# aipixel/GPS-Gaussian

Measured on NVIDIA H100. Metric: novel_views_per_sec_1024sq_500kgauss, higher is better.
Workload: dtype f32

## Files before the change

gps-gaussian_b200/csrc/gpsg_capi.cu:

```cuda
#include <cstdarg>
#include <cstdio>
#include <cstring>
#include <cstdlib>
#include "gpsg_internal.cuh"

namespace gpsg {

static thread_local char g_err[1024] = "";

void set_error(const char* fmt, ...) {
    va_list ap;
    va_start(ap, fmt);
    vsnprintf(g_err, sizeof(g_err), fmt, ap);
    va_end(ap);
}

Camera make_camera(const GpsgRasterSettings& s) {
    Camera c;
    memcpy(c.view, s.viewmatrix, sizeof(c.view));
    memcpy(c.proj, s.projmatrix, sizeof(c.proj));
    c.tanfovx = s.tanfovx;
    c.tanfovy = s.tanfovy;
    c.W = s.image_width;
    c.H = s.image_height;
    c.focal_x = (float)c.W / (2.0f * s.tanfovx);
    c.focal_y = (float)c.H / (2.0f * s.tanfovy);
    c.scale_modifier = s.scale_modifier;
    c.grid_x = (c.W + GPSG_TILE_X - 1) / GPSG_TILE_X;
    c.grid_y = (c.H + GPSG_TILE_Y - 1) / GPSG_TILE_Y;
    for (int k = 0; k < 3; ++k) { c.bg[k] = s.bg[k]; c.campos[k] = s.campos[k]; }
    return c;
}

template <typename T>
static inline T* take(char*& p, size_t count) {
    T* r = reinterpret_cast<T*>(p);
    p += align_up(count * sizeof(T));
    return r;
}

static GeomState carve_geom(char* p, int P, size_t scan_bytes, char** end) {
    GeomState g;
    const size_t n = (size_t)(P > 0 ? P : 1);
    g.depths = take<float>(p, n);
    g.means2D = take<float2>(p, n);
    g.conic_opacity = take<float4>(p, n);
    g.rgb = take<float>(p, 3 * n);
    g.clamped = take<uint8_t>(p, 3 * n);
    g.tiles_touched = take<uint32_t>(p, n);
    g.point_offsets = take<uint32_t>(p, n);
    g.scan_temp = p;
    g.scan_temp_bytes = scan_bytes;
    p += align_up(scan_bytes);
    if (end) *end = p;
    return g;
}
size_t GeomState::required(int P, size_t scan_bytes) {
    char* end = nullptr;
    carve_geom(nullptr, P, scan_bytes, &end);
    return (size_t)(end - (char*)nullptr) + 256;
}
GeomState GeomState::carve(void* base, int P, size_t scan_bytes) {
    return carve_geom((char*)align_up((size_t)base), P, scan_bytes, nullptr);
}

static BinningState carve_binning(char* p, size_t N, size_t sort_bytes, char** end) {
    BinningState b;
    const size_t n = N > 0 ? N : 1;
    b.slabA = take<float4>(p, n);
    b.slabB = take<float4>(p, n);
    b.slabC = take<float4>(p, n);
    b.keys = take<uint64_t>(p, n);
    b.vals = take<uint32_t>(p, n);
    b.keys_unsorted = take<uint64_t>(p, n);
    b.bucket = reinterpret_cast<uint2*>(b.keys_unsorted);
    b.vals_unsorted = take<uint32_t>(p, n);
    b.blk_list = take<uint32_t>(p, 8 * n);
    b.sort_temp = p;
    b.sort_temp_bytes = sort_bytes;
    p += align_up(sort_bytes);
    if (end) *end = p;
    return b;
}
size_t BinningState::required(size_t N, size_t sort_bytes) {
    char* end = nullptr;
    carve_binning(nullptr, N, sort_bytes, &end);
    return (size_t)(end - (char*)nullptr) + 256;
}
BinningState BinningState::carve(void* base, size_t N, size_t sort_bytes) {
    return carve_binning((char*)align_up((size_t)base), N, sort_bytes, nullptr);
}

static ImageState carve_image(char* p, int W, int H, char** end) {
    ImageState im;
    const size_t hw = (size_t)W * H;
    const size_t tiles = (size_t)((W + GPSG_TILE_X - 1) / GPSG_TILE_X) * ((H + GPSG_TILE_Y - 1) / GPSG_TILE_Y);
    im.final_T = take<float>(p, hw > 0 ? hw : 1);
    im.n_contrib = take<uint32_t>(p, hw > 0 ? hw : 1);
    im.ranges = take<uint2>(p, tiles > 0 ? tiles : 1);
    im.tile_count = take<uint32_t>(p, tiles > 0 ? tiles : 1);
    im.totals = take<uint32_t>(p, 64);
    im.tile_cursor = take<uint32_t>(p, tiles > 0 ? tiles : 1);
    im.big_tiles = take<uint32_t>(p, tiles > 0 ? tiles : 1);
    im.tile_order = take<uint32_t>(p, tiles > 0 ? tiles : 1);
    im.blk_count = take<uint32_t>(p, 8 * (tiles > 0 ? tiles : 1));
    if (end) *end = p;
    return im;
}
size_t ImageState::required(int W, int H) {
    char* end = nullptr;
    carve_image(nullptr, W, H, &end);
    return (size_t)(end - (char*)nullptr) + 256;
}
ImageState ImageState::carve(void* base, int W, int H) { return carve_image((char*)align_up((size_t)base), W, H, nullptr); }


static GaussianSrc aos_src(const float* means3D, const float* scales, const float* rots, const float* opacities,
                           const float* colors, const float* cov3D_precomp) {
    GaussianSrc src;
    memset(&src, 0, sizeof(src));
    src.means3D = means3D; src.scales = scales; src.rots = rots; src.opacities = opacities; src.colors = colors;
    src.cov3D_precomp = cov3D_precomp;
    return src;
}

static int bit_length(uint32_t n) {
    int b = 0;
    while (n) { ++b; n >>= 1; }
    return b;
}

static bool force_radix_binning() {
    static const bool v = [] { const char* e = getenv("GPSG_BINNING"); return e && e[0] == 'r'; }();
    return v;
}

static uint32_t* pinned_slot() {
    static thread_local uint32_t* slot = nullptr;
    if (!slot) {
        if (cudaHostAlloc((void**)&slot, 64, cudaHostAllocDefault) != cudaSuccess) slot = nullptr;
    }
    return slot;
}

}


#include <mutex>
#include <vector>
namespace gpsg {
struct ProfSlot { cudaEvent_t a, b; Stage stage; bool used; };
struct Profiler {
    int on = 0;
    std::vector<ProfSlot> slots;
    size_t next = 0;
    int launches[ST_COUNT] = {0};
};
static Profiler g_prof;
static std::mutex g_prof_mu;
static const char* kStageNames[ST_COUNT] = {"preprocess", "scan", "duplicate", "sort", "gather_ranges", "tile_scan",
                                            "bucket_scatter", "tile_sort_gather", "render_forward",
                                            "render_backward", "preprocess_backward", "corr_forward", "corr_backward", "corr_build",
                                            "render_backward_det", "render_backward_det_reduce"};
StageTimer::StageTimer(Stage s, cudaStream_t st, int launches) : stage(s), stream(st), slot(nullptr) {
    if (!g_prof.on) return;
    std::lock_guard<std::mutex> lk(g_prof_mu);
    if (g_prof.on == 2) { g_prof.launches[s] += launches; return; }
    if (g_prof.next == g_prof.slots.size()) {
        ProfSlot ps; ps.used = false;
        if (cudaEventCreate(&ps.a) != cudaSuccess || cudaEventCreate(&ps.b) != cudaSuccess) return;
        g_prof.slots.push_back(ps);
    }
    ProfSlot* p = &g_prof.slots[g_prof.next++];
    p->stage = s; p->used = true;
    g_prof.launches[s] += launches;
    cudaEventRecord(p->a, stream);
    slot = (void*)(uintptr_t)(g_prof.next);
}
StageTimer::~StageTimer() {
    if (!slot) return;
    std::lock_guard<std::mutex> lk(g_prof_mu);
    cudaEventRecord(g_prof.slots[(size_t)(uintptr_t)slot - 1].b, stream);
}
}

using namespace gpsg;

extern "C" {

GPSG_API const char* gpsg_last_error(void) { return g_err; }
int gpsg_version(void) { return 90; }

static int forward_exact_begin(const GpsgRasterSettings* s, int device, cudaStream_t stream, int P, const GaussianSrc& src,
                               int32_t* radii, gpsg_alloc_fn geom_alloc, void* geom_user, gpsg_alloc_fn image_alloc,
                               void* image_user, uint32_t* totals_host, void** geom_out, void** image_out, int flags) {
    GPSG_CUDA(cudaSetDevice(device));
    const Camera cam = make_camera(*s);
    const size_t scan_bytes = scan_temp_bytes(P);
    void* geom_base = geom_alloc(geom_user, GeomState::required(P, scan_bytes));
    if (!geom_base) { set_error("geometry allocator returned NULL"); return GPSG_E_ALLOC; }
    GeomState g = GeomState::carve(geom_base, P, scan_bytes);
    void* img_base = image_alloc(image_user, ImageState::required(cam.W, cam.H));
    if (!img_base) { set_error("image allocator returned NULL"); return GPSG_E_ALLOC; }
    ImageState im = ImageState::carve(img_base, cam.W, cam.H);
    if (geom_out) *geom_out = geom_base;
    if (image_out) *image_out = img_base;
    int rc = GPSG_OK;
    GPSG_CUDA(cudaMemsetAsync(im.tile_count, 0, (size_t)((char*)(im.totals + 64) - (char*)im.tile_count), stream));
    if (P > 0) {
        { StageTimer t(ST_PREPROCESS, stream, 1); rc = launch_preprocess(cam, P, src, radii, g, im, 0u, flags, stream); }
        if (rc) return rc;
        GPSG_CUDA(cudaMemcpyAsync(totals_host, im.totals, 6 * sizeof(uint32_t), cudaMemcpyDeviceToHost, stream));
    } else {
        { StageTimer t(ST_TILE_SCAN, stream, 1); rc = launch_tile_scan(cam, im, 0u, stream); }
        if (rc) return rc;
        for (int k = 0; k < 6; ++k) totals_host[k] = 0u;
    }
    return GPSG_OK;
}

static int forward_exact_finish(const GpsgRasterSettings* s, int device, cudaStream_t stream, int P, int sh_M, GaussianSrc src,
                                const float* shs, float* out_color, float* out_depth, float* out_alpha, int32_t* radii,
                                void* geom_base, void* img_base,
                                gpsg_alloc_fn binning_alloc, void* binning_user, const uint32_t* totals_host,
                                int32_t* num_rendered) {
    GPSG_CUDA(cudaSetDevice(device));
    const Camera cam = make_camera(*s);
    GeomState g = GeomState::carve(geom_base, P, scan_temp_bytes(P));
    ImageState im = ImageState::carve(img_base, cam.W, cam.H);
    const int tiles = cam.grid_x * cam.grid_y;
    const uint32_t N = totals_host[0], max_count = totals_host[1];
    GPSG_REQUIRE(totals_host[5] == 0u, "more than 2^31 (tile, Gaussian) pairs: the splats cover (almost) the whole image each -- "
                                       "degenerate scene (32-bit pair offsets, as in the upstream rasterizer)");
    int rc = GPSG_OK;
    if (num_rendered) *num_rendered = (int32_t)N;
    if (shs && P > 0) {
        rc = launch_sh_forward(P, s->sh_degree, sh_M, s->campos, src.means3D, shs, radii, g.rgb, g.clamped, stream);
        if (rc) return rc;
        src.colors = g.rgb;
    }

    const bool radix_path = max_count > kMaxTileSort || force_radix_binning();
    const int end_bit = 32 + bit_length((uint32_t)tiles);
    const size_t sort_bytes = radix_path ? sort_temp_bytes(N, end_bit) : 0;
    void* bin_base = binning_alloc(binning_user, BinningState::required(N, sort_bytes));
    if (!bin_base) { set_error("binning allocator returned NULL"); return GPSG_E_ALLOC; }
    BinningState b = BinningState::carve(bin_base, N, sort_bytes);

    if (N > 0 && !radix_path) {
        { StageTimer t(ST_SCATTER, stream, 1); rc = launch_bucket_scatter(cam, P, radii, g, b, im, stream); }
        if (rc) return rc;
        { StageTimer t(ST_TILE_SORT, stream, max_count > 2048 ? 2 : 1); rc = launch_tile_sort_gather(cam, P, max_count, src, g, b, im, stream); }
        if (rc) return rc;
    } else if (N > 0) {
        { StageTimer t(ST_SCAN, stream, 2); rc = run_scan(g, P, stream); }
        if (rc) return rc;
        { StageTimer t(ST_DUPLICATE, stream, 1); rc = launch_duplicate(cam, P, radii, g, b, stream); }
        if (rc) return rc;
        { StageTimer t(ST_SORT, stream, 2 + (end_bit + 7) / 8); rc = run_sort(b, N, end_bit, stream); }
        if (rc) return rc;
        { StageTimer t(ST_GATHER, stream, 2); rc = launch_gather_ranges(cam, N, src, g, b, im, stream); }
        if (rc) return rc;
    }
    { StageTimer t(ST_RENDER_FWD, stream, 1); rc = launch_render_forward(cam, b, im, out_color, g.depths, out_depth, out_alpha, stream); }
    if (rc) return rc;
    if (s->debug) GPSG_CUDA(cudaStreamSynchronize(stream));
    return GPSG_OK;
}

static int check_fwd_flags(int flags) {
    GPSG_REQUIRE((flags & ~GPSG_FWD_ANTIALIAS) == 0, "unknown forward flag bits (GPSG_FWD_ANTIALIAS is the only flag)");
    return GPSG_OK;
}

static int check_aux_outputs(const float* out_depth, const float* out_alpha) {
    GPSG_REQUIRE((out_depth == nullptr) == (out_alpha == nullptr), "out_depth and out_alpha must both be NULL or both be set");
    return GPSG_OK;
}

int gpsg_rasterize_forward(const GpsgRasterSettings* s, int device, void* stream_, int P, int sh_M,
                           const float* means3D, const float* colors_precomp, const float* shs,
                           const float* opacities, const float* scales, const float* rotations,
                           const float* cov3D_precomp, float* out_color, float* out_depth, float* out_alpha,
                           int32_t* radii, gpsg_alloc_fn geom_alloc, void* geom_user, gpsg_alloc_fn binning_alloc,
                           void* binning_user, gpsg_alloc_fn image_alloc, void* image_user, int32_t* num_rendered,
                           int flags) {
    if (int rc_f = check_fwd_flags(flags)) return rc_f;
    GPSG_REQUIRE(s != nullptr, "settings is NULL");
    GPSG_REQUIRE(P >= 0, "P < 0");
    GPSG_REQUIRE(s->image_width > 0 && s->image_height > 0, "image size must be positive");
    GPSG_REQUIRE(out_color != nullptr, "out_color is NULL");
    if (int rc_aux = check_aux_outputs(out_depth, out_alpha)) return rc_aux;
    GPSG_REQUIRE(geom_alloc && binning_alloc && image_alloc, "allocator callback is NULL");
    if (P > 0) {
        GPSG_REQUIRE(means3D && opacities && radii, "means3D / opacities / radii is NULL");
        GPSG_REQUIRE((colors_precomp != nullptr) != (shs != nullptr),
                     "Please provide excatly one of either SHs or precomputed colors!");
        GPSG_REQUIRE(((scales != nullptr && rotations != nullptr) != (cov3D_precomp != nullptr)),
                     "Please provide exactly one of either scale/rotation pair or precomputed 3D covariance!");
        if (shs) {
            GPSG_REQUIRE(s->sh_degree >= 0 && s->sh_degree <= 3, "sh_degree must be 0..3");
// ... 655 lines not shown
```

gps-gaussian_b200/csrc/gpsg_internal.cuh:

```cuda
#pragma once
#include <cuda_runtime.h>
#include <stdint.h>
#include <stddef.h>
#include "../../include/gpsg.h"

#define GPSG_TILE_X 16
#define GPSG_TILE_Y 16
#define GPSG_TILE_PIX 256

namespace gpsg {

void set_error(const char* fmt, ...);

#define GPSG_CUDA(expr)                                                                         \
    do {                                                                                        \
        cudaError_t _e = (expr);                                                                \
        if (_e != cudaSuccess) {                                                                \
            gpsg::set_error("%s:%d: %s -> %s", __FILE__, __LINE__, #expr, cudaGetErrorString(_e)); \
            return GPSG_E_CUDA;                                                                 \
        }                                                                                       \
    } while (0)
#define GPSG_LAUNCH_CHECK() GPSG_CUDA(cudaGetLastError())
#define GPSG_REQUIRE(cond, msg)                                  \
    do {                                                         \
        if (!(cond)) {                                           \
            gpsg::set_error("%s:%d: %s", __FILE__, __LINE__, msg); \
            return GPSG_E_INVALID;                               \
        }                                                        \
    } while (0)

struct Camera {
    float view[16];
    float proj[16];
    float tanfovx, tanfovy, focal_x, focal_y;
    float scale_modifier;
    int W, H, grid_x, grid_y;
    float bg[3];
    float campos[3];
};
Camera make_camera(const GpsgRasterSettings& s);


struct GaussianSrc {
    const float* means3D; const float* scales; const float* rots; const float* opacities; const float* colors;
    const float* cov3D_precomp;
    int S2;
    const uint8_t* valid[2]; const float* xyz[2]; const float* img[2]; const float* rot[2]; const float* scale[2];
    const float* opac[2];
};
struct GaussianGrads {
    float* dmeans3D; float* dscales; float* drots; float* dopacity; float* dcov3D;
    float* dxyz[2]; float* dimg[2]; float* drot[2]; float* dscale[2]; float* dopac[2];
};
#ifdef __CUDACC__
__device__ __forceinline__ bool src_geom(const GaussianSrc& s, int i, float& x, float& y, float& z, float sc[3], float4& q,
                                         float& op) {
    if (s.S2 == 0) {
        const float* m = s.means3D + 3 * (size_t)i;
        x = m[0]; y = m[1]; z = m[2];
        if (!s.cov3D_precomp) {
            const float* sp = s.scales + 3 * (size_t)i;
            sc[0] = sp[0]; sc[1] = sp[1]; sc[2] = sp[2];
            const float* rp = s.rots + 4 * (size_t)i;
            q = ((reinterpret_cast<uintptr_t>(s.rots) & 15) == 0) ? __ldg(reinterpret_cast<const float4*>(rp))
                                                                   : make_float4(rp[0], rp[1], rp[2], rp[3]);
        }
        op = s.opacities[i];
        return true;
    }
    const int v = i >= s.S2 ? 1 : 0, px = i - v * s.S2;
    if (!s.valid[v][px]) return false;
    const float* xyz = s.xyz[v] + 3 * (size_t)px;
    x = xyz[0]; y = xyz[1]; z = xyz[2];
    const size_t S2 = (size_t)s.S2;
    sc[0] = s.scale[v][px]; sc[1] = s.scale[v][S2 + px]; sc[2] = s.scale[v][2 * S2 + px];
    q = make_float4(s.rot[v][px], s.rot[v][S2 + px], s.rot[v][2 * S2 + px], s.rot[v][3 * S2 + px]);
    op = s.opac[v][px];
    return true;
}
__device__ __forceinline__ void tile_rect(int grid_x, int grid_y, float2 p, int radius, int& rx0, int& ry0, int& rx1,
                                          int& ry1) {
    const float rad = (float)radius;
    rx0 = min(grid_x, max(0, (int)((p.x - rad) / (float)GPSG_TILE_X)));
    ry0 = min(grid_y, max(0, (int)((p.y - rad) / (float)GPSG_TILE_Y)));
    rx1 = min(grid_x, max(0, (int)((p.x + rad + (float)(GPSG_TILE_X - 1)) / (float)GPSG_TILE_X)));
    ry1 = min(grid_y, max(0, (int)((p.y + rad + (float)(GPSG_TILE_Y - 1)) / (float)GPSG_TILE_Y)));
}
__device__ __forceinline__ int fwd_block_col(int k) { return (k >> 1) & 1; }
__device__ __forceinline__ int fwd_block_row(int k) { return ((k >> 2) << 1) + (k & 1); }
__device__ __forceinline__ void fwd_block_origin(int tile_x, int tile_y, int k, int& bx0, int& by0) {
    bx0 = tile_x * GPSG_TILE_X + (fwd_block_col(k) << 3);
    by0 = tile_y * GPSG_TILE_Y + (fwd_block_row(k) << 2);
}
__device__ __forceinline__ void src_color(const GaussianSrc& s, uint32_t id, float& r, float& g, float& b) {
    if (s.S2 == 0) { r = s.colors[3 * id]; g = s.colors[3 * id + 1]; b = s.colors[3 * id + 2]; return; }
    const int v = (int)id >= s.S2 ? 1 : 0;
    const size_t px = id - (uint32_t)(v * s.S2), S2 = (size_t)s.S2;
    r = s.img[v][px] * 0.5f + 0.5f; g = s.img[v][S2 + px] * 0.5f + 0.5f; b = s.img[v][2 * S2 + px] * 0.5f + 0.5f;
}
#endif

static inline size_t align_up(size_t v, size_t a = 256) { return (v + a - 1) / a * a; }

struct GeomState {
    float* depths;
    float2* means2D;
    float4* conic_opacity;
    float* rgb;
    uint8_t* clamped;
    uint32_t* tiles_touched;
    uint32_t* point_offsets;
    void* scan_temp;
    size_t scan_temp_bytes;
    static size_t required(int P, size_t scan_temp_bytes);
    static GeomState carve(void* base, int P, size_t scan_temp_bytes);
};
struct BinningState {
    uint2* bucket;
    uint64_t* keys_unsorted;
    uint32_t* vals_unsorted;
    uint64_t* keys;
    uint32_t* vals;
    float4* slabA;
    float4* slabB;
    float4* slabC;
    uint32_t* blk_list;
    void* sort_temp;
    size_t sort_temp_bytes;
    static size_t required(size_t N, size_t sort_temp_bytes);
    static BinningState carve(void* base, size_t N, size_t sort_temp_bytes);
};
struct ImageState {
    float* final_T;
    uint32_t* n_contrib;
    uint2* ranges;
    uint32_t* tile_count;
    uint32_t* tile_cursor;
    uint32_t* totals;
    uint32_t* big_tiles;
    uint32_t* tile_order;
    uint32_t* blk_count;
    static size_t required(int W, int H);
    static ImageState carve(void* base, int W, int H);
};
constexpr int kFwdFlagsWord = 6;
size_t scan_temp_bytes(int P);
size_t sort_temp_bytes(size_t N, int end_bit);

int launch_preprocess(const Camera& cam, int P, const GaussianSrc& src, int32_t* radii, GeomState g, ImageState im,
                      uint32_t capacity, int fwd_flags, cudaStream_t stream);
int launch_mark_visible(int P, const float* means3D, const float* view16_host, uint8_t* present, cudaStream_t stream);
int run_scan(GeomState g, int P, cudaStream_t stream);
int launch_duplicate(const Camera& cam, int P, const int32_t* radii, GeomState g, BinningState b, cudaStream_t stream);
int run_sort(BinningState b, size_t N, int end_bit, cudaStream_t stream);
int launch_gather_ranges(const Camera& cam, size_t N, const GaussianSrc& src, GeomState g, BinningState b, ImageState im,
                         cudaStream_t stream);
constexpr uint32_t kMaxTileSort = 4096;
int launch_tile_scan(const Camera& cam, ImageState im, uint32_t capacity , cudaStream_t stream);
int launch_bucket_scatter(const Camera& cam, int P, const int32_t* radii, GeomState g, BinningState b, ImageState im,
                          cudaStream_t stream);
int launch_tile_sort_gather(const Camera& cam, int P, uint32_t max_count, const GaussianSrc& src, GeomState g,
                            BinningState b, ImageState im, cudaStream_t stream);
int launch_render_forward(const Camera& cam, BinningState b, ImageState im, float* out_color, const float* depths,
                          float* out_depth, float* out_alpha, cudaStream_t stream);
struct AuxGrads {
    const float* depths; const float* dL_ddepth; const float* dL_dalpha;
    bool on() const { return dL_ddepth != nullptr; }
};
int launch_render_backward(const Camera& cam, BinningState b, ImageState im, const float* dL_dpix, float4* grad_acc,
                           const AuxGrads& aux, cudaStream_t stream);
int launch_render_backward_det(const Camera& cam, BinningState b, ImageState im, const float* dL_dpix, float* det_part,
                               uint32_t* det_mask, const AuxGrads& aux, cudaStream_t stream);
int launch_det_reduce(const Camera& cam, int P, const int32_t* radii, GeomState g, BinningState b, ImageState im,
                      const uint8_t* det_mask, const float* det_part, float4* grad_acc, bool aux, cudaStream_t stream);
int launch_preprocess_backward(const Camera& cam, int P, const GaussianSrc& src, const int32_t* radii,
                               const float4* conic_opacity, const uint32_t* fwd_flags ,
                               const float4* grad_acc, float* dL_dmeans2D ,
                               float* dL_dcolors , const GaussianGrads& out, bool aux,
                               cudaStream_t stream);
int launch_sh_forward(int P, int deg, int M, const float* campos3, const float* means3D, const float* shs,
                      const int32_t* radii, float* rgb, uint8_t* clamped, cudaStream_t stream);
int launch_sh_backward(int P, int deg, int M, const float* campos3, const float* means3D, const float* shs,
                       const int32_t* radii, const uint8_t* clamped, const float* dL_dcolors, float* dL_dsh,
                       float* dL_dmeans3D, cudaStream_t stream);
int launch_unproject_fwd(int B, int S, const float* flow, const float* mask, int64_t mask_bs, const float* intr,
                         const float* extr, int extr_rows, const float* ref_intr, const float* Tf_x, float* depth,
                         float* xyz, uint8_t* valid, cudaStream_t stream);
int launch_unproject_bwd(int B, int S, const float* depth, const float* mask, int64_t mask_bs, const float* intr,
                         const float* extr, int extr_rows, const float* ref_intr, const float* Tf_x,
                         const float* dL_dxyz, const float* dL_ddepth, float* dL_dflow, cudaStream_t stream);
struct RectifyView {
    double iR[9];
    double fx, fy, cx, cy;
    const uint8_t* img; const uint8_t* mask; const float* depth;
    uint8_t* img_out; uint8_t* mask_out; float* depth_out; float* img_tensor; float* mask_tensor;
};
struct RectifyArgs {
    RectifyView v[2];
    int Hin, Win, C, Cm, H, W;
};
struct RectifyFlowArgs {
    const float* depth[2]; const uint8_t* mask[2]; double* flow[2]; uint8_t* valid[2];
    double offset[2], tf[2];
    int H, W, Cm;
};
int launch_rectify_remap(const GpsgRectifyCamera* cams, int Hin, int Win, int C, int Cm, int H, int W,
                         const GpsgRectifyPlanes* planes, cudaStream_t stream);
int launch_rectify_flow(int H, int W, int Cm, double Tf_x, double cx0, double cx1, const float* const* depth,
                        const uint8_t* const* mask, double* const* flow, uint8_t* const* valid, cudaStream_t stream);
size_t point_splat_workspace_bytes(int B, int res);
int launch_point_splat(int B, int N, int res, int64_t rows, const float* pts, const float* mask, float* depth, float* color,
                       void* workspace, cudaStream_t stream);
size_t mesh_render_workspace_bytes(int num_faces, int64_t max_pixels);
int launch_mesh_render(const GpsgMesh& mesh, const GpsgMeshScene& scene, void* workspace, cudaStream_t stream);
int launch_convex_upsample_fwd(int dtype, int f, int N, int D, int H, int W, const float* flow, const void* mask, float* out,
                               cudaStream_t stream);
size_t convex_upsample_workspace_bytes(int N, int D, int H, int W);
int launch_convex_upsample_bwd(int dtype, int f, int N, int D, int H, int W, const float* flow, const void* mask,
                               const float* grad_out, void* grad_mask, float* grad_flow, void* workspace,
                               cudaStream_t stream);
size_t sequence_loss_workspace_bytes();
size_t gs_head_workspace_bytes(int B, int H, int W);
int launch_gs_head_fwd(int device, int B, int H, int W, const float* src, const float* img, const float* depth,
                       const GpsgGsHeadWeights& wt, float* rot, float* scale, float* opacity, void* workspace,
                       cudaStream_t stream);
size_t gs_head_backward_workspace_bytes(int B, int H, int W);
int launch_gs_head_bwd(int device, int B, int H, int W, const float* src, const float* img, const float* depth,
                       const float* mid, const float* g_rot, const float* g_scale, const float* g_opacity,
                       const GpsgGsHeadWeights& wt, float* d_src, float* d_depth, const GpsgGsHeadGrads& grads,
                       void* workspace, cudaStream_t stream);
int launch_sequence_loss_fwd(const GpsgSeqLossArgs& a, float* stats, void* workspace, cudaStream_t stream);
int launch_sequence_loss_bwd(const GpsgSeqLossArgs& a, const float* grad_loss, const float* stats, cudaStream_t stream);
int corr_build_mode();
void set_corr_build_mode(int m);
int launch_corr_fwd(int dtype, int B, int H, int W1, int W2, const void* vol, int64_t sb, int64_t sh, int64_t sw1,
                    const float* coords, int64_t csb, int r, void* out, cudaStream_t stream);
int launch_corr_bwd(int dtype, int B, int H, int W1, int W2, const float* coords, int64_t csb, const void* gout, int r,
                    void* gvol, cudaStream_t stream);
int launch_corr_build(int dtype, int B, int D, int H, int W1, int W2, const void* f1, const void* f2, void* v0, void* v1,
                      void* v2, void* v3, int levels, cudaStream_t stream);
bool corr_build_tc_supported(int dtype, int D, int W1, int W2, const void* f1, const void* f2, void* const* v, int levels);
int launch_corr_build_tc(int B, int D, int H, int W1, int W2, const void* f1, const void* f2, void* v0, void* v1, void* v2,
                         void* v3, int levels, cudaStream_t stream);
bool corr_build_bwd_tc_supported(int dtype, int D, int W1, int W2, const void* f1, const void* f2, const void* g,
                                 const void* d1, const void* d2);
int launch_corr_build_bwd_tc(int B, int D, int H, int W1, int W2, const void* f1, const void* f2, const void* g, void* df1,
                             void* df2, cudaStream_t stream);
int launch_corr_build_bwd(int dtype, int B, int D, int H, int W1, int W2, const void* f1, const void* f2, const void* g,
                          void* df1, void* df2, cudaStream_t stream);
int launch_corr_lookup_fwd(int dtype, int B, int H, int W1, const void* const* vols, const int* widths, int levels,
                           const float* coords, int64_t csb, int r, void* out, cudaStream_t stream);
int launch_corr_lookup_bwd(int dtype, int B, int H, int W1, void* const* gvols, const int* widths, int levels,
                           const float* coords, int64_t csb, int r, const void* gout, cudaStream_t stream);

size_t l1_ssim_workspace_bytes(int planes, int H, int W);
int launch_l1_ssim_fwd(int planes, int H, int W, const float* img, const float* gt, float w_l1, float w_ssim, float* out3,
                       float* dmaps, void* workspace, cudaStream_t stream);
int launch_l1_ssim_bwd(int planes, int H, int W, const float* img, const float* gt, const float* dmaps, float w_l1,
                       float w_ssim, const float* grad_loss, float* dimg, cudaStream_t stream);

enum Stage { ST_PREPROCESS = 0, ST_SCAN, ST_DUPLICATE, ST_SORT, ST_GATHER, ST_TILE_SCAN, ST_SCATTER, ST_TILE_SORT, ST_RENDER_FWD, ST_RENDER_BWD,
             ST_PREPROCESS_BWD, ST_CORR_FWD, ST_CORR_BWD, ST_CORR_BUILD, ST_RENDER_BWD_DET, ST_RENDER_BWD_DET_REDUCE, ST_COUNT };
struct StageTimer {
    StageTimer(Stage s, cudaStream_t stream, int launches);
    ~StageTimer();
    Stage stage; cudaStream_t stream; void* slot;
};

}
```

gps-gaussian_b200/csrc/raster_binning.cu:

```cuda
#include <cub/cub.cuh>
#include "gpsg_internal.cuh"
#include "tile_scan.cuh"

namespace gpsg {

size_t scan_temp_bytes(int P) {
    size_t bytes = 0;
    cub::DeviceScan::InclusiveSum(nullptr, bytes, (uint32_t*)nullptr, (uint32_t*)nullptr, P > 0 ? P : 1);
    return bytes;
}

size_t sort_temp_bytes(size_t N, int end_bit) {
    size_t bytes = 0;
    cub::DeviceRadixSort::SortPairs(nullptr, bytes, (uint64_t*)nullptr, (uint64_t*)nullptr, (uint32_t*)nullptr,
                                    (uint32_t*)nullptr, (int64_t)(N > 0 ? N : 1), 0, end_bit);
    return bytes;
}

int run_scan(GeomState g, int P, cudaStream_t stream) {
    if (P <= 0) return GPSG_OK;
    size_t bytes = g.scan_temp_bytes;
    GPSG_CUDA(cub::DeviceScan::InclusiveSum(g.scan_temp, bytes, g.tiles_touched, g.point_offsets, P, stream));
    return GPSG_OK;
}

__global__ void __launch_bounds__(256) duplicate_kernel(const __grid_constant__ Camera cam, int P,
                                                        const int32_t* __restrict__ radii, GeomState g,
                                                        BinningState b) {
    const int i = blockIdx.x * blockDim.x + threadIdx.x;
    if (i >= P) return;
    const int radius = radii[i];
    if (radius <= 0) return;
    uint32_t off = (i == 0) ? 0u : g.point_offsets[i - 1];
    int rx0, ry0, rx1, ry1;
    tile_rect(cam.grid_x, cam.grid_y, g.means2D[i], radius, rx0, ry0, rx1, ry1);
    const uint64_t dbits = (uint64_t)__float_as_uint(g.depths[i]);
    for (int y = ry0; y < ry1; ++y)
        for (int x = rx0; x < rx1; ++x) {
            const uint64_t key = ((uint64_t)(uint32_t)(y * cam.grid_x + x) << 32) | dbits;
            b.keys_unsorted[off] = key;
            b.vals_unsorted[off] = (uint32_t)i;
            ++off;
        }
}

int launch_duplicate(const Camera& cam, int P, const int32_t* radii, GeomState g, BinningState b, cudaStream_t stream) {
    if (P <= 0) return GPSG_OK;
    duplicate_kernel<<<(P + 255) / 256, 256, 0, stream>>>(cam, P, radii, g, b);
    GPSG_LAUNCH_CHECK();
    return GPSG_OK;
}

int run_sort(BinningState b, size_t N, int end_bit, cudaStream_t stream) {
    if (N == 0) return GPSG_OK;
    size_t bytes = b.sort_temp_bytes;
    GPSG_CUDA(cub::DeviceRadixSort::SortPairs(b.sort_temp, bytes, b.keys_unsorted, b.keys, b.vals_unsorted, b.vals,
                                              (int64_t)N, 0, end_bit, stream));
    return GPSG_OK;
}



__global__ void __launch_bounds__(256) tile_scan_kernel(int tiles, ImageState im, uint32_t capacity) {
    tile_scan_block(tiles, im, capacity);
}

int launch_tile_scan(const Camera& cam, ImageState im, uint32_t capacity, cudaStream_t stream) {
    tile_scan_kernel<<<1, 256, 0, stream>>>(cam.grid_x * cam.grid_y, im, capacity);
    GPSG_LAUNCH_CHECK();
    return GPSG_OK;
}

__global__ void __launch_bounds__(256) bucket_scatter_kernel(const __grid_constant__ Camera cam, int P,
                                                             const int32_t* __restrict__ radii, GeomState g,
                                                             BinningState b, ImageState im) {
    __shared__ uint32_t sh_cnt[kBoxBins];
    __shared__ uint32_t sh_base[kBoxBins];
    __shared__ int s_bb[4];
    if (im.totals[2]) return;
    if (threadIdx.x == 0) { s_bb[0] = 0x7fffffff; s_bb[1] = 0x7fffffff; s_bb[2] = 0; s_bb[3] = 0; }
    for (int t = threadIdx.x; t < kBoxBins; t += blockDim.x) sh_cnt[t] = 0u;
    __syncthreads();
    const int i = blockIdx.x * blockDim.x + threadIdx.x;
    int rx0 = 0, ry0 = 0, rx1 = 0, ry1 = 0;
    uint2 entry = make_uint2(0u, 0u);
    if (i < P) {
        const int radius = radii[i];
        if (radius > 0) {
            tile_rect(cam.grid_x, cam.grid_y, g.means2D[i], radius, rx0, ry0, rx1, ry1);
            entry = make_uint2((uint32_t)i, __float_as_uint(g.depths[i]));
        }
    }
    TileBox box;
    if (!cta_tile_box(rx0, ry0, rx1, ry1, s_bb, box)) {
        for (int y = ry0; y < ry1; ++y)
            for (int x = rx0; x < rx1; ++x) {
                const int t = y * cam.grid_x + x;
                b.bucket[im.ranges[t].x + atomicAdd(&im.tile_cursor[t], 1u)] = entry;
            }
        return;
    }
    for (int y = ry0; y < ry1; ++y)
        for (int x = rx0; x < rx1; ++x) atomicAdd(&sh_cnt[(y - box.y0) * box.w + (x - box.x0)], 1u);
    __syncthreads();
    for (int t = threadIdx.x; t < box.w * box.h; t += blockDim.x) {
        const uint32_t c = sh_cnt[t];
        if (c) {
            const int tile = (box.y0 + t / box.w) * cam.grid_x + box.x0 + t % box.w;
            sh_base[t] = im.ranges[tile].x + atomicAdd(&im.tile_cursor[tile], c);
            sh_cnt[t] = 0u;
        }
    }
    __syncthreads();
    for (int y = ry0; y < ry1; ++y)
        for (int x = rx0; x < rx1; ++x) {
            const int t = (y - box.y0) * box.w + (x - box.x0);
            b.bucket[sh_base[t] + atomicAdd(&sh_cnt[t], 1u)] = entry;
        }
}

int launch_bucket_scatter(const Camera& cam, int P, const int32_t* radii, GeomState g, BinningState b, ImageState im,
                          cudaStream_t stream) {
    if (P <= 0) return GPSG_OK;
    bucket_scatter_kernel<<<(P + 255) / 256, 256, 0, stream>>>(cam, P, radii, g, b, im);
    GPSG_LAUNCH_CHECK();
    return GPSG_OK;
}

__device__ __forceinline__ void slab_entry(uint32_t id, const GaussianSrc& src, const GeomState& g, float4& A,
                                           float4& B, float4& C) {
    const float2 xy = g.means2D[id];
    const float4 co = g.conic_opacity[id];
    float r, gg, bb;
    src_color(src, id, r, gg, bb);
    float ex = 3.0e38f, ey = 3.0e38f;
    const float detc = co.x * co.z - co.y * co.y;
    if (!(co.w * 255.0f >= 1.0f)) {
        ex = ey = -3.0e38f;
    } else if (detc > 0.0f && co.x > 0.0f && co.z > 0.0f) {
        const float tau2 = 2.0f * __logf(co.w * 255.0f) * 1.0005f + 1e-4f;
        ex = sqrtf(tau2 * co.z / detc) * 1.0005f + 0.01f;
        ey = sqrtf(tau2 * co.x / detc) * 1.0005f + 0.01f;
        if (!(ex == ex) || !(ey == ey)) { ex = 3.0e38f; ey = 3.0e38f; }
    }
    A = make_float4(xy.x, xy.y, ex, ey);
    const float kL = 1.4426950408889634f;
    B = make_float4(-0.5f * kL * co.x, -kL * co.y, -0.5f * kL * co.z, co.w);
    C = make_float4(r, gg, bb, __uint_as_float(id));
}

constexpr int kSortThreads = 512;
constexpr int kSortWarps = kSortThreads / 32;
constexpr int kSortCTAsPerSM = 3;

struct BlockLists {
    uint32_t cnt[kSortWarps][8];
    uint32_t off[kSortWarps][8];
    uint32_t base[8];
};

__device__ __forceinline__ void build_block_lists(BlockLists& s, const float4* __restrict__ tileA, uint32_t n, int tile_x,
                                                  int tile_y, uint32_t* __restrict__ list, uint32_t* __restrict__ count) {
    const int lane = threadIdx.x & 31, warp = threadIdx.x >> 5;
    const unsigned lt = (1u << lane) - 1u;
    float wx0[2], wx1[2], wy0[4], wy1[4];
#pragma unroll
    for (int k = 0; k < 8; ++k) {
        int bx0, by0;
        fwd_block_origin(tile_x, tile_y, k, bx0, by0);
        wx0[fwd_block_col(k)] = (float)bx0; wx1[fwd_block_col(k)] = (float)(bx0 + 7);
        wy0[fwd_block_row(k)] = (float)by0; wy1[fwd_block_row(k)] = (float)(by0 + 3);
    }
    if (threadIdx.x < 8) s.base[threadIdx.x] = 0u;
#pragma unroll 1
    for (uint32_t c0 = 0; c0 < n; c0 += kSortThreads) {
        const uint32_t r = c0 + threadIdx.x;
        const bool valid = r < n;
        const float4 a = valid ? tileA[r] : make_float4(0.f, 0.f, 0.f, 0.f);
        bool hx[2], hy[4];
#pragma unroll
        for (int c = 0; c < 2; ++c) hx[c] = (a.x >= wx0[c] - a.z) && (a.x <= wx1[c] + a.z);
#pragma unroll
        for (int w = 0; w < 4; ++w) hy[w] = (a.y >= wy0[w] - a.w) && (a.y <= wy1[w] + a.w);
        uint32_t hits = 0u;
#pragma unroll
        for (int k = 0; k < 8; ++k) {
            const bool hit = valid && hx[fwd_block_col(k)] && hy[fwd_block_row(k)];
            hits |= (uint32_t)hit << k;
            const unsigned m = __ballot_sync(0xffffffffu, hit);
            if (lane == k) s.cnt[warp][k] = __popc(m);
        }
        __syncthreads();
        if (threadIdx.x < kSortWarps * 8) {
            static_assert(kSortWarps == 16, "one 16-lane segment per block");
            const int k = threadIdx.x >> 4, w = threadIdx.x & 15;
            const uint32_t cw = s.cnt[w][k];
            uint32_t incl = cw;
#pragma unroll
            for (int o = 1; o < 16; o <<= 1) {
                const uint32_t u = __shfl_up_sync(0xffffffffu, incl, o, 16);
                if (w >= o) incl += u;
            }
            const uint32_t b = s.base[k];
            s.off[w][k] = b + incl - cw;
            __syncwarp();
            if (w == 15) s.base[k] = b + incl;
        }
        __syncthreads();
#pragma unroll
        for (int k = 0; k < 8; ++k) {
            const unsigned m = __ballot_sync(0xffffffffu, (hits >> k) & 1u);
            if ((hits >> k) & 1u) list[(size_t)k * n + s.off[warp][k] + __popc(m & lt)] = r;
        }
    }
    if (threadIdx.x < 8) count[threadIdx.x] = s.base[threadIdx.x];
}

constexpr int kBigItems = (int)kMaxTileSort / kSortThreads;
template <int ITEMS>
struct TileSort {
    using BRS = cub::BlockRadixSort<uint32_t, kSortThreads, ITEMS, uint32_t, 4, false>;
    union Smem {
        typename BRS::TempStorage sort;
        unsigned long long keys[kSortThreads * ITEMS];
    };

    static constexpr int kMaxRun = 16;
    __device__ static void run(Smem& sm, uint32_t* flags, BlockLists& bl, const uint2* __restrict__ src, int n, int id_bits,
                               uint32_t tile, int grid_x, size_t out0, const GaussianSrc& src_in, const GeomState& g,
                               const BinningState& b, uint32_t* __restrict__ blk_count) {
        uint32_t keys[ITEMS], ids[ITEMS];
        uint32_t dmin = ~0u, dmax = 0u;
#pragma unroll
        for (int k = 0; k < ITEMS; ++k) {
            const int i = k * kSortThreads + (int)threadIdx.x;
            const uint2 e = i < n ? src[i] : make_uint2(0u, 0u);
            ids[k] = e.x;
            keys[k] = e.y;
            if (i < n) { dmin = min(dmin, e.y); dmax = max(dmax, e.y); }
        }
        dmin = __reduce_min_sync(0xffffffffu, dmin);
        dmax = __reduce_max_sync(0xffffffffu, dmax);
        if (threadIdx.x == 0) { flags[0] = ~0u; flags[1] = 0u; flags[2] = 0u; }
        __syncthreads();
        if ((threadIdx.x & 31) == 0) { atomicMin(&flags[0], dmin); atomicMax(&flags[1], dmax); }
        __syncthreads();
        const uint32_t dlo = flags[0];
        const int w = 32 - __clz(flags[1] - dlo);
        const uint32_t pad = 1u << w;
#pragma unroll
        for (int k = 0; k < ITEMS; ++k) keys[k] = (k * kSortThreads + (int)threadIdx.x) < n ? keys[k] - dlo : pad;
        BRS(sm.sort).SortBlockedToStriped(keys, ids, 0, w + 1);
        __syncthreads();
#pragma unroll
        for (int k = 0; k < ITEMS; ++k)
            sm.keys[k * kSortThreads + (int)threadIdx.x] = ((unsigned long long)(keys[k] + dlo) << 32) | ids[k];
        __syncthreads();
        bool redo = false;
#pragma unroll 1
        for (int k = 0; k < ITEMS; ++k) {
            const int r = k * kSortThreads + (int)threadIdx.x;
            if (r + 1 < n) {
                const uint32_t d = (uint32_t)(sm.keys[r] >> 32);
                const bool start = (r == 0 || (uint32_t)(sm.keys[r - 1] >> 32) != d) && (uint32_t)(sm.keys[r + 1] >> 32) == d;
                if (start) {
                    int e = r + 1;
                    while (e + 1 < n && (uint32_t)(sm.keys[e + 1] >> 32) == d) ++e;
                    if (e - r + 1 > kMaxRun) redo = true;
                    else
                        for (int a = r + 1; a <= e; ++a) {
                            const unsigned long long v = sm.keys[a];
                            int c = a - 1;
                            while (c >= r && sm.keys[c] > v) { sm.keys[c + 1] = sm.keys[c]; --c; }
                            sm.keys[c + 1] = v;
                        }
                }
            }
        }
        if (redo) flags[2] = 1u;
        __syncthreads();
        if (flags[2]) {
#pragma unroll
            for (int k = 0; k < ITEMS; ++k) {
                const int r = k * kSortThreads + (int)threadIdx.x;
                const unsigned long long v = sm.keys[r];
                ids[k] = (uint32_t)v;
                keys[k] = r < n ? (uint32_t)(v >> 32) - dlo : pad;
            }
            __syncthreads();
            BRS(sm.sort).SortBlockedToStriped(ids, keys, 0, id_bits);
            __syncthreads();
#pragma unroll
            for (int k = 0; k < ITEMS; ++k)
                sm.keys[k * kSortThreads + (int)threadIdx.x] = ((unsigned long long)keys[k] << 32) | ids[k];
            __syncthreads();
#pragma unroll
            for (int k = 0; k < ITEMS; ++k) {
                const unsigned long long v = sm.keys[(int)threadIdx.x * ITEMS + k];
                ids[k] = (uint32_t)v;
                keys[k] = (uint32_t)(v >> 32);
            }
            __syncthreads();
            BRS(sm.sort).SortBlockedToStriped(keys, ids, 0, w + 1);
            __syncthreads();
#pragma unroll
            for (int k = 0; k < ITEMS; ++k)
                sm.keys[k * kSortThreads + (int)threadIdx.x] = ((unsigned long long)(keys[k] + dlo) << 32) | ids[k];
            __syncthreads();
        }
        const unsigned long long tile_hi = (unsigned long long)tile << 32;
#pragma unroll 1
        for (int k = 0; k < ITEMS; ++k) {
            const int r = k * kSortThreads + (int)threadIdx.x;
            if (r < n) {
                const unsigned long long v = sm.keys[r];
                const uint32_t id = (uint32_t)v;
                const size_t o = out0 + r;
                if (b.keys) {
                    b.keys[o] = tile_hi | (v >> 32);
                    b.vals[o] = id;
                }
                float4 A, B, C;
                slab_entry(id, src_in, g, A, B, C);
                b.slabA[o] = A;
                b.slabB[o] = B;
                b.slabC[o] = C;
            }
        }
        const int tile_y = (int)tile / grid_x;
        build_block_lists(bl, b.slabA + out0, (uint32_t)n, (int)tile - tile_y * grid_x, tile_y, b.blk_list + 8 * out0,
                          blk_count + 8 * (size_t)tile);
    }
};

template <bool BIG>
__global__ void __launch_bounds__(kSortThreads, BIG ? 1 : kSortCTAsPerSM) tile_sort_gather_kernel(const GaussianSrc colors, GeomState g,
                                                                            BinningState b, ImageState im, int id_bits,
                                                                            int grid_x) {
    __shared__ uint32_t flags[4];
    __shared__ BlockLists bl;
    if (im.totals[2]) return;
    if constexpr (BIG) {
        __shared__ typename TileSort<kBigItems>::Smem t16;
        const uint32_t nbig = im.totals[3];
        for (uint32_t k = blockIdx.x; k < nbig; k += gridDim.x) {
            const uint32_t tile = im.big_tiles[k];
            const uint2 range = im.ranges[tile];
            const int n = (int)(range.y - range.x);
            TileSort<kBigItems>::run(t16, flags, bl, b.bucket + range.x, n, id_bits, tile, grid_x, range.x, colors, g, b,
                                     im.blk_count);
            __syncthreads();
        }
    } else {
        __shared__ union {
            typename TileSort<1>::Smem t1;
            typename TileSort<2>::Smem t2;
            typename TileSort<3>::Smem t3;
            typename TileSort<4>::Smem t4;
        } temp;
        const uint32_t tile = im.tile_order[blockIdx.x];
        const uint2 range = im.ranges[tile];
        const int n = (int)(range.y - range.x);
        if (n == 0 || n > (int)kBigTile) return;
        const uint2* __restrict__ src = b.bucket + range.x;
        if (n <= 512) TileSort<1>::run(temp.t1, flags, bl, src, n, id_bits, tile, grid_x, range.x, colors, g, b, im.blk_count);
        else if (n <= 1024) TileSort<2>::run(temp.t2, flags, bl, src, n, id_bits, tile, grid_x, range.x, colors, g, b, im.blk_count);
        else if (n <= 1536) TileSort<3>::run(temp.t3, flags, bl, src, n, id_bits, tile, grid_x, range.x, colors, g, b, im.blk_count);
        else TileSort<4>::run(temp.t4, flags, bl, src, n, id_bits, tile, grid_x, range.x, colors, g, b, im.blk_count);
    }
}

constexpr int kBigTileCTAs = 132;

int launch_tile_sort_gather(const Camera& cam, int P, uint32_t max_count, const GaussianSrc& colors, GeomState g,
                            BinningState b, ImageState im, cudaStream_t stream) {
    int id_bits = 1;
    while (id_bits < 32 && (1ll << id_bits) < (long long)P) ++id_bits;
    const int tiles = cam.grid_x * cam.grid_y;
    tile_sort_gather_kernel<false><<<tiles, kSortThreads, 0, stream>>>(colors, g, b, im, id_bits, cam.grid_x);
    GPSG_LAUNCH_CHECK();
    if (max_count > kBigTile) {
        tile_sort_gather_kernel<true><<<min(tiles, kBigTileCTAs), kSortThreads, 0, stream>>>(colors, g, b, im, id_bits,
                                                                                             cam.grid_x);
        GPSG_LAUNCH_CHECK();
    }
    return GPSG_OK;
}

__global__ void __launch_bounds__(256) gather_ranges_kernel(size_t N, const GaussianSrc colors, GeomState g,
                                                            BinningState b, ImageState im) {
    const size_t i = (size_t)blockIdx.x * blockDim.x + threadIdx.x;
    if (i >= N) return;
    const uint64_t key = b.keys[i];
    const uint32_t tile = (uint32_t)(key >> 32);
    if (i == 0) {
        im.ranges[tile].x = 0;
    } else {
        const uint32_t prev = (uint32_t)(b.keys[i - 1] >> 32);
        if (prev != tile) {
            im.ranges[prev].y = (uint32_t)i;
            im.ranges[tile].x = (uint32_t)i;
        }
    }
    if (i == N - 1) im.ranges[tile].y = (uint32_t)N;
    const uint32_t id = b.vals[i];
    float4 A, B, C;
    slab_entry(id, colors, g, A, B, C);
    b.slabA[i] = A;
    b.slabB[i] = B;
    b.slabC[i] = C;
}

__global__ void __launch_bounds__(kSortThreads) block_lists_kernel(int grid_x, BinningState b, ImageState im) {
    __shared__ BlockLists bl;
    const uint32_t tile = blockIdx.x;
    const uint2 range = im.ranges[tile];
    const uint32_t n = range.y - range.x;
    if (n == 0) return;
    const int tile_y = (int)tile / grid_x;
    build_block_lists(bl, b.slabA + range.x, n, (int)tile - tile_y * grid_x, tile_y, b.blk_list + 8 * (size_t)range.x,
                      im.blk_count + 8 * (size_t)tile);
}

int launch_gather_ranges(const Camera& cam, size_t N, const GaussianSrc& colors, GeomState g, BinningState b, ImageState im,
                         cudaStream_t stream) {
    const int tiles = cam.grid_x * cam.grid_y;
    GPSG_CUDA(cudaMemsetAsync(im.ranges, 0, sizeof(uint2) * (size_t)tiles, stream));
    if (N == 0) return GPSG_OK;
    gather_ranges_kernel<<<(unsigned)((N + 255) / 256), 256, 0, stream>>>(N, colors, g, b, im);
    GPSG_LAUNCH_CHECK();
    block_lists_kernel<<<tiles, kSortThreads, 0, stream>>>(cam.grid_x, b, im);
    GPSG_LAUNCH_CHECK();
    return GPSG_OK;
}

}
```

Baseline: 5074.

## Use persistent ticket scheduling for tile sort and split block-list building across warps

```diff
diff --git a/gps-gaussian_b200/csrc/gpsg_capi.cu b/gps-gaussian_b200/csrc/gpsg_capi.cu
--- a/gps-gaussian_b200/csrc/gpsg_capi.cu
+++ b/gps-gaussian_b200/csrc/gpsg_capi.cu
@@ -2,6 +2,9 @@
 #include <cstdio>
 #include <cstring>
 #include <cstdlib>
+#include <map>
+#include <mutex>
+#include <utility>
 #include "gpsg_internal.cuh"
 
 namespace gpsg {
@@ -13,6 +16,22 @@
     va_start(ap, fmt);
     vsnprintf(g_err, sizeof(g_err), fmt, ap);
     va_end(ap);
+}
+
+int resident_grid(const void* kernel, int threads) {
+    static std::mutex mu;
+    static std::map<std::pair<int, const void*>, int> cache;
+    int dev = 0;
+    if (cudaGetDevice(&dev) != cudaSuccess) return -1;
+    std::lock_guard<std::mutex> lk(mu);
+    const auto key = std::make_pair(dev, kernel);
+    const auto it = cache.find(key);
+    if (it != cache.end()) return it->second;
+    int per_sm = 0, sms = 0;
+    if (cudaOccupancyMaxActiveBlocksPerMultiprocessor(&per_sm, kernel, threads, 0) != cudaSuccess ||
+        cudaDeviceGetAttribute(&sms, cudaDevAttrMultiProcessorCount, dev) != cudaSuccess || per_sm < 1 || sms < 1)
+        return -1;
+    return cache[key] = per_sm * sms;
 }
 
 Camera make_camera(const GpsgRasterSettings& s) {
@@ -146,7 +165,6 @@
 }
 
 
-#include <mutex>
 #include <vector>
 namespace gpsg {
 struct ProfSlot { cudaEvent_t a, b; Stage stage; bool used; };
diff --git a/gps-gaussian_b200/csrc/gpsg_internal.cuh b/gps-gaussian_b200/csrc/gpsg_internal.cuh
--- a/gps-gaussian_b200/csrc/gpsg_internal.cuh
+++ b/gps-gaussian_b200/csrc/gpsg_internal.cuh
@@ -39,6 +39,7 @@
     float campos[3];
 };
 Camera make_camera(const GpsgRasterSettings& s);
+int resident_grid(const void* kernel, int threads);
 
 
 struct GaussianSrc {
@@ -144,6 +145,7 @@
     static ImageState carve(void* base, int W, int H);
 };
 constexpr int kFwdFlagsWord = 6;
+constexpr int kSortTicketWord = 7;
 size_t scan_temp_bytes(int P);
 size_t sort_temp_bytes(size_t N, int end_bit);
 
diff --git a/gps-gaussian_b200/csrc/raster_binning.cu b/gps-gaussian_b200/csrc/raster_binning.cu
--- a/gps-gaussian_b200/csrc/raster_binning.cu
+++ b/gps-gaussian_b200/csrc/raster_binning.cu
@@ -150,70 +150,39 @@
 }
 
 constexpr int kSortThreads = 512;
-constexpr int kSortWarps = kSortThreads / 32;
 constexpr int kSortCTAsPerSM = 3;
 
-struct BlockLists {
-    uint32_t cnt[kSortWarps][8];
-    uint32_t off[kSortWarps][8];
-    uint32_t base[8];
-};
-
-__device__ __forceinline__ void build_block_lists(BlockLists& s, const float4* __restrict__ tileA, uint32_t n, int tile_x,
-                                                  int tile_y, uint32_t* __restrict__ list, uint32_t* __restrict__ count) {
-    const int lane = threadIdx.x & 31, warp = threadIdx.x >> 5;
+
+__device__ __forceinline__ uint32_t block_hit_mask(const float4& a, int tile_x, int tile_y) {
+    bool hx[2], hy[4];
+#pragma unroll
+    for (int c = 0; c < 2; ++c) {
+        const float wx0 = (float)(tile_x * GPSG_TILE_X + 8 * c), wx1 = (float)(tile_x * GPSG_TILE_X + 8 * c + 7);
+        hx[c] = (a.x >= wx0 - a.z) && (a.x <= wx1 + a.z);
+    }
+#pragma unroll
+    for (int w = 0; w < 4; ++w) {
+        const float wy0 = (float)(tile_y * GPSG_TILE_Y + 4 * w), wy1 = (float)(tile_y * GPSG_TILE_Y + 4 * w + 3);
+        hy[w] = (a.y >= wy0 - a.w) && (a.y <= wy1 + a.w);
+    }
+    uint32_t hits = 0u;
+#pragma unroll
+    for (int k = 0; k < 8; ++k) hits |= (uint32_t)(hx[fwd_block_col(k)] && hy[fwd_block_row(k)]) << k;
+    return hits;
+}
+
+__device__ __forceinline__ void append_block_list(const uint8_t* hits, uint32_t r0, uint32_t m, int k,
+                                                  uint32_t* __restrict__ list, uint32_t& base) {
+    const int lane = threadIdx.x & 31;
     const unsigned lt = (1u << lane) - 1u;
-    float wx0[2], wx1[2], wy0[4], wy1[4];
-#pragma unroll
-    for (int k = 0; k < 8; ++k) {
-        int bx0, by0;
-        fwd_block_origin(tile_x, tile_y, k, bx0, by0);
-        wx0[fwd_block_col(k)] = (float)bx0; wx1[fwd_block_col(k)] = (float)(bx0 + 7);
-        wy0[fwd_block_row(k)] = (float)by0; wy1[fwd_block_row(k)] = (float)(by0 + 3);
-    }
-    if (threadIdx.x < 8) s.base[threadIdx.x] = 0u;
-#pragma unroll 1
-    for (uint32_t c0 = 0; c0 < n; c0 += kSortThreads) {
-        const uint32_t r = c0 + threadIdx.x;
-        const bool valid = r < n;
-        const float4 a = valid ? tileA[r] : make_float4(0.f, 0.f, 0.f, 0.f);
-        bool hx[2], hy[4];
-#pragma unroll
-        for (int c = 0; c < 2; ++c) hx[c] = (a.x >= wx0[c] - a.z) && (a.x <= wx1[c] + a.z);
-#pragma unroll
-        for (int w = 0; w < 4; ++w) hy[w] = (a.y >= wy0[w] - a.w) && (a.y <= wy1[w] + a.w);
-        uint32_t hits = 0u;
-#pragma unroll
-        for (int k = 0; k < 8; ++k) {
-            const bool hit = valid && hx[fwd_block_col(k)] && hy[fwd_block_row(k)];
-            hits |= (uint32_t)hit << k;
-            const unsigned m = __ballot_sync(0xffffffffu, hit);
-            if (lane == k) s.cnt[warp][k] = __popc(m);
-        }
-        __syncthreads();
-        if (threadIdx.x < kSortWarps * 8) {
-            static_assert(kSortWarps == 16, "one 16-lane segment per block");
-            const int k = threadIdx.x >> 4, w = threadIdx.x & 15;
-            const uint32_t cw = s.cnt[w][k];
-            uint32_t incl = cw;
-#pragma unroll
-            for (int o = 1; o < 16; o <<= 1) {
-                const uint32_t u = __shfl_up_sync(0xffffffffu, incl, o, 16);
-                if (w >= o) incl += u;
-            }
-            const uint32_t b = s.base[k];
-            s.off[w][k] = b + incl - cw;
-            __syncwarp();
-            if (w == 15) s.base[k] = b + incl;
-        }
-        __syncthreads();
-#pragma unroll
-        for (int k = 0; k < 8; ++k) {
-            const unsigned m = __ballot_sync(0xffffffffu, (hits >> k) & 1u);
-            if ((hits >> k) & 1u) list[(size_t)k * n + s.off[warp][k] + __popc(m & lt)] = r;
-        }
-    }
-    if (threadIdx.x < 8) count[threadIdx.x] = s.base[threadIdx.x];
+#pragma unroll 4
+    for (uint32_t c = 0; c < m; c += 32) {
+        const uint32_t i = c + lane;
+        const bool hit = i < m && ((hits[i] >> k) & 1u);
+        const unsigned mask = __ballot_sync(0xffffffffu, hit);
+        if (hit) list[base + __popc(mask & lt)] = r0 + i;
+        base += __popc(mask);
+    }
 }
 
 constexpr int kBigItems = (int)kMaxTileSort / kSortThreads;
@@ -226,7 +195,7 @@
     };
 
     static constexpr int kMaxRun = 16;
-    __device__ static void run(Smem& sm, uint32_t* flags, BlockLists& bl, const uint2* __restrict__ src, int n, int id_bits,
+    __device__ static void run(Smem& sm, uint32_t* flags, uint8_t* hits, const uint2* __restrict__ src, int n, int id_bits,
                                uint32_t tile, int grid_x, size_t out0, const GaussianSrc& src_in, const GeomState& g,
                                const BinningState& b, uint32_t* __restrict__ blk_count) {
         uint32_t keys[ITEMS], ids[ITEMS];
@@ -309,6 +278,7 @@
             __syncthreads();
         }
         const unsigned long long tile_hi = (unsigned long long)tile << 32;
+        const int tile_y = (int)tile / grid_x, tile_x = (int)tile - tile_y * grid_x;
 #pragma unroll 1
         for (int k = 0; k < ITEMS; ++k) {
             const int r = k * kSortThreads + (int)threadIdx.x;
@@ -325,29 +295,42 @@
                 b.slabA[o] = A;
                 b.slabB[o] = B;
                 b.slabC[o] = C;
+                hits[r] = (uint8_t)block_hit_mask(A, tile_x, tile_y);
             }
         }
-        const int tile_y = (int)tile / grid_x;
-        build_block_lists(bl, b.slabA + out0, (uint32_t)n, (int)tile - tile_y * grid_x, tile_y, b.blk_list + 8 * out0,
-                          blk_count + 8 * (size_t)tile);
+        __syncthreads();
+        const int warp = (int)threadIdx.x >> 5, blk = warp & 7;
+        const uint32_t split = ((uint32_t)n / 2u) & ~127u;
+        uint32_t* __restrict__ list = b.blk_list + 8 * out0 + (size_t)blk * n;
+        uint32_t cnt = 0u;
+        if (warp < 8) {
+            append_block_list(hits, 0u, split, blk, list, cnt);
+        } else {
+            const uint32_t* __restrict__ words = reinterpret_cast<const uint32_t*>(hits);
+#pragma unroll 1
+            for (uint32_t i = threadIdx.x & 31; i < split / 4u; i += 32) cnt += __popc(words[i] & (0x01010101u << blk));
+            cnt = __reduce_add_sync(0xffffffffu, cnt);
+            append_block_list(hits + split, split, (uint32_t)n - split, blk, list, cnt);
+            if ((threadIdx.x & 31) == 0) blk_count[8 * (size_t)tile + blk] = cnt;
+        }
     }
 };
 
 template <bool BIG>
 __global__ void __launch_bounds__(kSortThreads, BIG ? 1 : kSortCTAsPerSM) tile_sort_gather_kernel(const GaussianSrc colors, GeomState g,
                                                                             BinningState b, ImageState im, int id_bits,
-                                                                            int grid_x) {
+                                                                            int grid_x, uint32_t tiles) {
     __shared__ uint32_t flags[4];
-    __shared__ BlockLists bl;
     if (im.totals[2]) return;
     if constexpr (BIG) {
         __shared__ typename TileSort<kBigItems>::Smem t16;
+        __shared__ __align__(16) uint8_t hits[kSortThreads * kBigItems];
         const uint32_t nbig = im.totals[3];
         for (uint32_t k = blockIdx.x; k < nbig; k += gridDim.x) {
             const uint32_t tile = im.big_tiles[k];
             const uint2 range = im.ranges[tile];
             const int n = (int)(range.y - range.x);
-            TileSort<kBigItems>::run(t16, flags, bl, b.bucket + range.x, n, id_bits, tile, grid_x, range.x, colors, g, b,
+            TileSort<kBigItems>::run(t16, flags, hits, b.bucket + range.x, n, id_bits, tile, grid_x, range.x, colors, g, b,
                                      im.blk_count);
             __syncthreads();
         }
@@ -358,15 +341,24 @@
             typename TileSort<3>::Smem t3;
             typename TileSort<4>::Smem t4;
         } temp;
-        const uint32_t tile = im.tile_order[blockIdx.x];
-        const uint2 range = im.ranges[tile];
-        const int n = (int)(range.y - range.x);
-        if (n == 0 || n > (int)kBigTile) return;
-        const uint2* __restrict__ src = b.bucket + range.x;
-        if (n <= 512) TileSort<1>::run(temp.t1, flags, bl, src, n, id_bits, tile, grid_x, range.x, colors, g, b, im.blk_count);
-        else if (n <= 1024) TileSort<2>::run(temp.t2, flags, bl, src, n, id_bits, tile, grid_x, range.x, colors, g, b, im.blk_count);
-        else if (n <= 1536) TileSort<3>::run(temp.t3, flags, bl, src, n, id_bits, tile, grid_x, range.x, colors, g, b, im.blk_count);
-        else TileSort<4>::run(temp.t4, flags, bl, src, n, id_bits, tile, grid_x, range.x, colors, g, b, im.blk_count);
+        __shared__ __align__(16) uint8_t hits[kSortThreads * 4];
+#pragma unroll 1
+        for (;;) {
+            if (threadIdx.x == 0) flags[3] = atomicAdd(&im.totals[kSortTicketWord], 1u);
+            __syncthreads();
+            const uint32_t i = flags[3];
+            if (i >= tiles) break;
+            const uint32_t tile = im.tile_order[i];
+            const uint2 range = im.ranges[tile];
+            const int n = (int)(range.y - range.x);
+            if (n == 0) break;
+            const uint2* __restrict__ src = b.bucket + range.x;
+            if (n <= 512) TileSort<1>::run(temp.t1, flags, hits, src, n, id_bits, tile, grid_x, range.x, colors, g, b, im.blk_count);
+            else if (n <= 1024) TileSort<2>::run(temp.t2, flags, hits, src, n, id_bits, tile, grid_x, range.x, colors, g, b, im.blk_count);
+            else if (n <= 1536) TileSort<3>::run(temp.t3, flags, hits, src, n, id_bits, tile, grid_x, range.x, colors, g, b, im.blk_count);
+            else if (n <= (int)kBigTile) TileSort<4>::run(temp.t4, flags, hits, src, n, id_bits, tile, grid_x, range.x, colors, g, b, im.blk_count);
+            __syncthreads();
+        }
     }
 }
 
@@ -377,11 +369,14 @@
     int id_bits = 1;
     while (id_bits < 32 && (1ll << id_bits) < (long long)P) ++id_bits;
     const int tiles = cam.grid_x * cam.grid_y;
-    tile_sort_gather_kernel<false><<<tiles, kSortThreads, 0, stream>>>(colors, g, b, im, id_bits, cam.grid_x);
+    const int ctas = resident_grid((const void*)tile_sort_gather_kernel<false>, kSortThreads);
+    GPSG_REQUIRE(ctas > 0, "tile sort: could not query the occupancy of tile_sort_gather_kernel on the current device");
+    tile_sort_gather_kernel<false><<<min(tiles, ctas), kSortThreads, 0, stream>>>(colors, g, b, im, id_bits, cam.grid_x,
+                                                                                   (uint32_t)tiles);
     GPSG_LAUNCH_CHECK();
     if (max_count > kBigTile) {
         tile_sort_gather_kernel<true><<<min(tiles, kBigTileCTAs), kSortThreads, 0, stream>>>(colors, g, b, im, id_bits,
-                                                                                             cam.grid_x);
+                                                                                             cam.grid_x, (uint32_t)tiles);
         GPSG_LAUNCH_CHECK();
     }
     return GPSG_OK;
@@ -411,15 +406,27 @@
     b.slabC[i] = C;
 }
 
+constexpr uint32_t kListChunk = 8 * kSortThreads;
 __global__ void __launch_bounds__(kSortThreads) block_lists_kernel(int grid_x, BinningState b, ImageState im) {
-    __shared__ BlockLists bl;
+    __shared__ uint8_t hits[kListChunk];
     const uint32_t tile = blockIdx.x;
     const uint2 range = im.ranges[tile];
     const uint32_t n = range.y - range.x;
     if (n == 0) return;
-    const int tile_y = (int)tile / grid_x;
-    build_block_lists(bl, b.slabA + range.x, n, (int)tile - tile_y * grid_x, tile_y, b.blk_list + 8 * (size_t)range.x,
-                      im.blk_count + 8 * (size_t)tile);
+    const int tile_y = (int)tile / grid_x, tile_x = (int)tile - tile_y * grid_x;
+    const float4* __restrict__ tileA = b.slabA + range.x;
+    const int warp = (int)threadIdx.x >> 5;
+    uint32_t* __restrict__ list = b.blk_list + 8 * (size_t)range.x + (size_t)min(warp, 7) * n;
+    uint32_t cnt = 0u;
+#pragma unroll 1
+    for (uint32_t r0 = 0; r0 < n; r0 += kListChunk) {
+        const uint32_t m = min(kListChunk, n - r0);
+        for (uint32_t i = threadIdx.x; i < m; i += kSortThreads) hits[i] = (uint8_t)block_hit_mask(tileA[r0 + i], tile_x, tile_y);
+        __syncthreads();
+        if (warp < 8) append_block_list(hits, r0, m, warp, list, cnt);
+        __syncthreads();
+    }
+    if (warp < 8 && (threadIdx.x & 31) == 0) im.blk_count[8 * (size_t)tile + warp] = cnt;
 }
 
 int launch_gather_ranges(const Camera& cam, size_t N, const GaussianSrc& colors, GeomState g, BinningState b, ImageState im,
```

After: 5263, median of 6. 3.7% higher.
